# jhoobergs/Thesis-pbrt-v3

Measured on AMD Instinct MI355X. Metric: Mrays/s, higher is better.
Workload: dtype f32; 1 GPU; Sponza-class atrium STAND-IN (311,728 tris, matte+plastic, point light; the reference ships no Sponza geometry) 700x700, halton 1024 spp, path maxdepth 5, bvh; spp_total=1024, tiles=16x16 round-robin over 1 GPU(s), parallelism=tile-dp1, film_merge=none (single GPU)

## Files before the change

thesis-pbrt-v3_amd/csrc/capi_device.hip:

```cpp
#include <hip/hip_runtime.h>
#include <algorithm>
#include <chrono>
#include <cmath>
#include <cstring>
#include <functional>
#include <map>
#include <memory>
#include <string>
#include <vector>
#include "../../include/hprt.h"
#include "device/kernels.h"
#include "halton_tables.h"
#include "host_transform.h"
#include "hprt_internal.h"
#include "device_state.h"
#include "scene_layout.h"
#include "wide_bvh.h"

using namespace hprt;


namespace {

int CheckDevice(int device, int *chosen) {
// ... 179 lines not shown
        dv.voxFunc = sc->voxFunc.as<float>(); dv.voxCdf = sc->voxCdf.as<float>(); dv.voxFuncInt = sc->voxFuncInt.as<float>();
        sc->nVoxels = (uint32_t)nVox; sc->voxRows = (uint32_t)rows; sc->voxRowsUsed = 0;
        if (dense) LaunchVoxelDistributions(nullptr, dv, sc->voxRi.as<float>(), (uint32_t)nVox, sc->voxFunc.as<float>(), sc->voxCdf.as<float>(), sc->voxFuncInt.as<float>());
        else {
            HIP_TRY(sc->voxSlot.alloc(nVox * sizeof(int32_t)));
            HIP_TRY(hipMemset(sc->voxSlot.p, 0xff, nVox * sizeof(int32_t)));
            HIP_TRY(sc->voxRequest.alloc(nVox * sizeof(uint32_t)));
            HIP_TRY(sc->voxRequestCount.alloc(256));
            HIP_TRY(hipMemset(sc->voxRequestCount.p, 0, 256));
            dv.voxSlot = sc->voxSlot.as<int32_t>(); dv.voxRequest = sc->voxRequest.as<uint32_t>(); dv.voxRequestCount = sc->voxRequestCount.as<uint32_t>();
        }
        HIP_TRY(hipGetLastError());
        HIP_TRY(hipDeviceSynchronize());
    }
    HIP_TRY(hipHostMalloc((void **)&sc->hostCounts, (4096 + 256) * sizeof(uint32_t)));
    *out = sc.release();
    return HPRT_OK;
} catch (...) { return hprt::HandleException(); }

__attribute__((visibility("default"))) int hprt_debug_scene_walk(HprtScene *s) { return s && s->walk == HprtScene::Walk::Bvh && hprt::WideWalkInUse(s->dev) ? 1 : 0; }
__attribute__((visibility("default"))) int hprt_debug_shade_counts(HprtScene *s, int on, uint64_t *out2) {
    if (!s) return HPRT_E_INVALID;
    if (out2) { out2[0] = s->shadeDeferred; out2[1] = s->shadeRetried; }
    if (on && !s->shadeCountsOn) s->shadeDeferred = s->shadeRetried = 0;
    s->shadeCountsOn = on != 0;
    return HPRT_OK;
}
__attribute__((visibility("default"))) int hprt_debug_poison_workspace(HprtScene *s, int byte) { if (!s) return HPRT_E_INVALID; s->poisonByte = byte < 0 ? -1 : (byte & 255); return HPRT_OK; }
__attribute__((visibility("default"))) int hprt_debug_capture_rays(HprtScene *s, int bounce, int kind, float *d_out7, size_t cap) {
    if (!s || kind < 0 || kind > 2 || cap > 0x7fffffffull) return HPRT_E_INVALID;
    s->capture.bounce = bounce; s->capture.kind = kind; s->capture.out7 = d_out7; s->capture.cap = cap; s->capture.n = 0;
    return HPRT_OK;
}
static int ApiStreams(HprtScene *s, size_t n, RayStream *rays, HitStream *hits);
static bool CountsKdShare(const HprtScene *s) { return s->walk == HprtScene::Walk::RbspKd || s->walk == HprtScene::Walk::BspPaperKd; }
static void Trace(HprtScene *s, hipStream_t st, bool anyHit, bool count, const uint32_t *queue, const uint32_t *countPtr, uint32_t countImm,
                  uint32_t gridItems, const RayStream &rays, const HitStream &hits, uint8_t *occ, DevCounters *counters, uint32_t *workCounter,
                  uint4 *rayStats = nullptr) {
    switch (s->walk) {
    case HprtScene::Walk::Kd: LaunchKdTrace(st, s->dev, s->kd, anyHit, count, queue, countPtr, countImm, gridItems, rays, hits, occ, counters, workCounter, rayStats); break;
    case HprtScene::Walk::Rbsp: LaunchRbspTrace(st, s->dev, s->rbsp, anyHit, count, queue, countPtr, countImm, gridItems, rays, hits, occ, counters, workCounter, rayStats); break;
    case HprtScene::Walk::RbspKd:
        LaunchRbspKdTrace(st, s->dev, DevRbspKd{s->rbsp, s->kdShare.as<unsigned long long>()}, anyHit, count, queue, countPtr, countImm, gridItems, rays,
                          hits, occ, counters, workCounter, rayStats);
        break;
    case HprtScene::Walk::BspPaper:
        LaunchBspPaperTrace(st, s->dev, s->bsppaper, anyHit, count, queue, countPtr, countImm, gridItems, rays, hits, occ, counters, workCounter, rayStats);
        break;
    case HprtScene::Walk::BspPaperKd:
        LaunchBspPaperKdTrace(st, s->dev, DevBspPaperKd{s->bsppaper, s->kdShare.as<unsigned long long>()}, anyHit, count, queue, countPtr, countImm,
// ... 403 lines not shown
        HIP_TRY(outOcc.alloc(n));
        HitStream none; none.a = nullptr; none.b = nullptr;
        Trace(s, nullptr, true, count, nullptr, nullptr, (uint32_t)n, (uint32_t)n, rays, none, outOcc.as<uint8_t>(), s->counters.as<DevCounters>(), s->workCounter.as<uint32_t>());
        HIP_TRY(hipGetLastError()); HIP_TRY(hipDeviceSynchronize());
        if (occ_out) HIP_TRY(hipMemcpy(occ_out, outOcc.p, n, hipMemcpyDeviceToHost));
    }
    if (counters) ReadCounters(s, anyHit, counters);
    return HPRT_OK;
}
int hprt_intersect(HprtScene *s, size_t n, const float *o, const float *d, const float *tmax, float *t_out, int32_t *prim_out,
                   float *bary_out, uint64_t counters[4]) try {
    return TraceHost(s, false, n, o, d, tmax, t_out, prim_out, nullptr, bary_out, nullptr, counters);
} catch (...) { return hprt::HandleException(); }
int hprt_intersect_instanced(HprtScene *s, size_t n, const float *o, const float *d, const float *tmax, float *t_out, int32_t *prim_out,
                             int32_t *inst_out, float *bary_out, uint64_t counters[4]) try {
    return TraceHost(s, false, n, o, d, tmax, t_out, prim_out, inst_out, bary_out, nullptr, counters);
} catch (...) { return hprt::HandleException(); }
int hprt_occluded(HprtScene *s, size_t n, const float *o, const float *d, const float *tmax, uint8_t *occ, uint64_t counters[4]) try {
    return TraceHost(s, true, n, o, d, tmax, nullptr, nullptr, nullptr, nullptr, occ, counters);
} catch (...) { return hprt::HandleException(); }

namespace {

struct BatchTimers { double extendMs = 0, occludedMs = 0; uint64_t extendLaunches = 0, occludedLaunches = 0, extendRays = 0, occludedRays = 0; };

int RunBatch(HprtScene *s, hipStream_t st, const RenderParams &rp, const Workspace &w, const QueueSet &qa, const QueueSet &qb,
             const BinSet &bins, uint32_t s0, uint32_t nSlots, bool count, EventTimer &ev, BatchTimers *bt, HprtRenderStats *stats,
             uint32_t *pixelStats = nullptr, const IrregularSink *irregular = nullptr) {
    uint4 *rayStats = pixelStats ? s->rayStats.as<uint4>() : nullptr;
    uint32_t *pixelKd = pixelStats && CountsKdShare(s) ? s->pixelKdLocal.as<uint32_t>() : nullptr;
    uint32_t *wcPath = s->workCounter.as<uint32_t>();
    LaunchGenerate(st, s->dev, rp, w.path[0], s0, nSlots, irregular);
    const uint32_t *activeQ = nullptr; uint32_t active = nSlots;
    QueueSet q[2] = {qa, qb};
    DevCounters *ctr = s->counters.as<DevCounters>();
    std::vector<std::pair<hipEvent_t, hipEvent_t>> evExt, evOcc;
    auto tracePath = [&](int bounce) -> int {
        const PathStream &in = w.path[bounce & 1];
        hipEvent_t e0 = ev.get(), e1 = ev.get();
        HIP_TRY(hipEventRecord(e0, st));
        Trace(s, st, false, count, activeQ, nullptr, active, active, in.ray, w.hit, nullptr, ctr, wcPath, rayStats);
        if (pixelStats) LaunchPixelStats(st, rayStats, bounce == 0 ? nullptr : in.beta, activeQ, nullptr, active, active, rp.nPix, false, pixelStats);
        if (pixelKd) LaunchPixelKdStats(st, rayStats, bounce == 0 ? nullptr : in.beta, activeQ, nullptr, active, active, rp.nPix, false, pixelKd);
        HIP_TRY(hipEventRecord(e1, st));
        evExt.push_back({e0, e1}); bt->extendRays += active; ++bt->extendLaunches;
        stats->rays += active;
        return HPRT_OK;
    };
    if (active > 0) { int rc = tracePath(0); if (rc != HPRT_OK) return rc; }
    for (int bounce = 0; active > 0; ++bounce) {
        const QueueSet &cur = q[bounce & 1];
        const PathStream &in = w.path[bounce & 1], &out = w.path[(bounce + 1) & 1];
// ... 44 lines not shown
            hipEvent_t a = ev.get(), b = ev.get();
            HIP_TRY(hipEventRecord(a, st));
            HitStream none; none.a = nullptr; none.b = nullptr;
            Trace(s, st, true, count, cur.shadow, nullptr, nShadow, nShadow, w.vs.shadow, none, w.vs.occluded, ctr, wcPath, rayStats);
            if (pixelStats) LaunchPixelStats(st, rayStats, w.vs.pendBeta, cur.shadow, nullptr, nShadow, nShadow, rp.nPix, true, pixelStats);
            if (pixelKd) LaunchPixelKdStats(st, rayStats, w.vs.pendBeta, cur.shadow, nullptr, nShadow, nShadow, rp.nPix, true, pixelKd);
            HIP_TRY(hipEventRecord(b, st));
            evOcc.push_back({a, b}); bt->occludedRays += nShadow; ++bt->occludedLaunches;
            stats->shadow_rays += nShadow;
        }
        if (nMis) {
            hipEvent_t a = ev.get(), b = ev.get();
            HIP_TRY(hipEventRecord(a, st));
            Trace(s, st, false, count, cur.mis, nullptr, nMis, nMis, w.vs.mis, w.vs.misHit, nullptr, ctr, wcPath, rayStats);
            if (pixelStats) LaunchPixelStats(st, rayStats, w.vs.pendBeta, cur.mis, nullptr, nMis, nMis, rp.nPix, false, pixelStats);
            if (pixelKd) LaunchPixelKdStats(st, rayStats, w.vs.pendBeta, cur.mis, nullptr, nMis, nMis, rp.nPix, false, pixelKd);
            HIP_TRY(hipEventRecord(b, st));
            evExt.push_back({a, b}); bt->extendRays += nMis; ++bt->extendLaunches;
            stats->rays += nMis;
        }
        activeQ = cur.next; active = nNext;
        if (active > 0 && bounce > rp.maxDepth) return SetError(HPRT_E_DEVICE, "internal error: paths are still active beyond maxdepth");
        if (nResolve) LaunchResolve(st, s->dev, w.vs, out.L, w.Lfinal, cur.resolve, cur.resolveCount, nResolve);
        if (active > 0) { int rc = tracePath(bounce + 1); if (rc != HPRT_OK) return rc; }
    }
    HIP_TRY(hipGetLastError());
    HIP_TRY(hipStreamSynchronize(st));
    for (auto &p : evExt) { float ms = 0; if (hipEventElapsedTime(&ms, p.first, p.second) == hipSuccess) bt->extendMs += ms; }
    for (auto &p : evOcc) { float ms = 0; if (hipEventElapsedTime(&ms, p.first, p.second) == hipSuccess) bt->occludedMs += ms; }
    ev.reset();
    return HPRT_OK;
}

constexpr size_t kQueueWordsPerSlot = 8 + 1 + 2 * N_BINS;
int EnsureWorkspace(HprtScene *s, size_t nSlots, Workspace *ps, QueueSet *qa, QueueSet *qb, BinSet *bins) {
    HIP_TRY(s->planes.alloc(PlaneBytes(nSlots)));
    CarvePlanes(s->planes.as<char>(), nSlots, ps);
    HIP_TRY(s->queues.alloc(kQueueWordsPerSlot * nSlots * sizeof(uint32_t) + 4096));
    HIP_TRY(s->queueCounts.alloc(2048 * sizeof(uint32_t)));
    uint32_t *qbase = s->queues.as<uint32_t>(), *cbase = s->queueCounts.as<uint32_t>();
    QueueSet *qs[2] = {qa, qb};
    for (int k = 0; k < 2; ++k) {
        qs[k]->next = qbase + (4 * k + 0) * nSlots; qs[k]->shadow = qbase + (4 * k + 1) * nSlots;
        qs[k]->mis = qbase + (4 * k + 2) * nSlots; qs[k]->resolve = qbase + (4 * k + 3) * nSlots;
        qs[k]->nextCount = cbase + 256 * k; qs[k]->shadowCount = cbase + 256 * k + 64; qs[k]->misCount = cbase + 256 * k + 128; qs[k]->resolveCount = cbase + 256 * k + 192;
    }
    bins->aux = qbase + 8 * nSlots;
    for (int k = 0; k < (int)N_BINS; ++k) bins->q[k] = reinterpret_cast<uint2 *>(qbase + (9 + 2 * k) * nSlots + (nSlots & 1u));
    bins->count = cbase + 512;
    bins->retry[0] = bins->retry[1] = nullptr;
// ... 69 lines not shown
    HIP_TRY(hipMemsetAsync(film, 0, 16 * s->filmPixels, st));
    if (nPix == 0) { HIP_TRY(hipStreamSynchronize(st)); return HPRT_OK; }
    const size_t lallBytes = 3ull * spp * nPix * sizeof(float);
    if (lallBytes > (96ull << 30)) return SetError(HPRT_E_UNSUPPORTED, "per-sample radiance store would exceed 96 GiB; render in several tile ranges");
    uint32_t chunk = 0;
    if ((rc = ChooseBatch(s, desc->spp_chunk, nPix, spp, &chunk)) != HPRT_OK) return rc;
    const size_t maxSlots = (size_t)chunk * nPix;
    Workspace ps; QueueSet qa, qb; BinSet bins;
    rc = EnsureWorkspace(s, maxSlots, &ps, &qa, &qb, &bins);
    if (rc != HPRT_OK) return rc;
    HIP_TRY(s->Lall.alloc(lallBytes));
    if ((rc = PoisonWorkspace(s)) != HPRT_OK) return rc;
    float *LallR = s->Lall.as<float>(), *LallG = LallR + (size_t)spp * nPix, *LallB = LallG + (size_t)spp * nPix;
    HIP_TRY(upload(s->pixelXY, f.pixelXY)); HIP_TRY(upload(s->pixelOffset, f.pixelOffset));
    RenderParams rp;
    MakeCamera(o, &rp.cam);
    rp.hal.baseScale1 = f.hal.baseScales[1]; rp.hal.baseExp0 = f.hal.baseExponents[0]; rp.hal.sampleStride = f.hal.sampleStride;
    rp.hal.samplePixelCenter = o.sample_pixel_center;
    rp.pixelXY = s->pixelXY.as<uint32_t>(); rp.pixelOffset = s->pixelOffset.as<uint64_t>(); rp.nPix = nPix;
    rp.maxDepth = o.max_depth; rp.rrThreshold = o.rr_threshold;
    rp.invSqrtSpp = 1 / std::sqrt((float)spp);
    const bool wantPixelStats = (desc->flags & HPRT_RENDER_PIXEL_STATS) != 0;
    const bool count = (desc->flags & HPRT_RENDER_COUNT_WORK) != 0 || wantPixelStats;
    rp.cullMis = (!count || (desc->flags & HPRT_RENDER_COUNT_TRACED) != 0) && !(desc->flags & HPRT_RENDER_TRACE_ALL) ? 1 : 0;
    uint32_t *pixelStats = nullptr;
    if (wantPixelStats) {
        HIP_TRY(s->rayStats.alloc(sizeof(uint4) * maxSlots));
        HIP_TRY(s->pixelStatsLocal.alloc(6ull * nPix * sizeof(uint32_t)));
        HIP_TRY(hipMemsetAsync(s->pixelStatsLocal.p, 0, 6ull * nPix * sizeof(uint32_t), st));
        HIP_TRY(s->pixelStatsFilm.alloc(7ull * s->filmPixels * sizeof(uint64_t)));
        HIP_TRY(hipMemsetAsync(s->pixelStatsFilm.p, 0, 7ull * s->filmPixels * sizeof(uint64_t), st));
        pixelStats = s->pixelStatsLocal.as<uint32_t>();
        if (CountsKdShare(s)) {
            HIP_TRY(s->pixelKdLocal.alloc(2ull * nPix * sizeof(uint32_t)));
            HIP_TRY(hipMemsetAsync(s->pixelKdLocal.p, 0, 2ull * nPix * sizeof(uint32_t), st));
            HIP_TRY(s->pixelKdFilm.alloc(2ull * s->filmPixels * sizeof(uint64_t)));
            HIP_TRY(hipMemsetAsync(s->pixelKdFilm.p, 0, 2ull * s->filmPixels * sizeof(uint64_t), st));
        }
    }
    s->pixelStatsValid = false; s->pixelKdValid = false;
    HIP_TRY(hipMemsetAsync(s->counters.p, 0, sizeof(DevCounters), st));
    if (CountsKdShare(s)) HIP_TRY(hipMemsetAsync(s->kdShare.p, 0, 2 * sizeof(unsigned long long), st));

    auto wall0 = std::chrono::high_resolution_clock::now();
    static const uint32_t capHint = [] { const char *e = getenv("HPRT_IRREGULAR_CAP"); return e ? (uint32_t)std::max(1, atoi(e)) : (1u << 24); }();
    uint32_t irrCap = (uint32_t)std::min<uint64_t>((uint64_t)nPix * spp, capHint);
// ... 183 lines not shown
    SceneCall call(s, nullptr);
    FrameSetup f;
    int rc = SetupFrame(*opt, &f);
    if (rc != HPRT_OK) return rc;
    std::vector<uint32_t> xy(n); std::vector<uint64_t> off(n);
    for (size_t i = 0; i < n; ++i) {
        if (px[i] < f.fg.sx0 || px[i] >= f.fg.sx1 || py[i] < f.fg.sy0 || py[i] >= f.fg.sy1 || sample[i] < 0)
            return SetError(HPRT_E_INVALID, "hprt_sample_radiance: pixel outside the sample bounds");
        xy[i] = (uint32_t)px[i] | ((uint32_t)py[i] << 16);
        off[i] = (uint64_t)HaltonPixelOffset(f.hal, px[i], py[i]) + (uint64_t)sample[i] * (uint64_t)f.hal.sampleStride;
    }
    Workspace ps; QueueSet qa, qb; BinSet bins;
    rc = EnsureWorkspace(s, n, &ps, &qa, &qb, &bins);
    if (rc != HPRT_OK) return rc;
    HIP_TRY(upload(s->pixelXY, xy)); HIP_TRY(upload(s->pixelOffset, off));
    HIP_TRY(s->Lall.alloc(12 * n));
    if ((rc = PoisonWorkspace(s)) != HPRT_OK) return rc;
    RenderParams rp;
    MakeCamera(*opt, &rp.cam);
    rp.hal.baseScale1 = f.hal.baseScales[1]; rp.hal.baseExp0 = f.hal.baseExponents[0]; rp.hal.sampleStride = f.hal.sampleStride;
    rp.hal.samplePixelCenter = opt->sample_pixel_center;
    rp.pixelXY = s->pixelXY.as<uint32_t>(); rp.pixelOffset = s->pixelOffset.as<uint64_t>(); rp.nPix = (uint32_t)n;
    rp.maxDepth = opt->max_depth; rp.rrThreshold = opt->rr_threshold;
    rp.invSqrtSpp = 1 / std::sqrt((float)std::max(1, opt->spp)); rp.cullMis = 1;
    EventTimer ev; BatchTimers bt; HprtRenderStats stats; memset(&stats, 0, sizeof(stats));
    rc = RunBatch(s, nullptr, rp, ps, qa, qb, bins, 0, (uint32_t)n, false, ev, &bt, &stats);
    if (rc != HPRT_OK) return rc;
    float *LR = s->Lall.as<float>();
    LaunchStoreRadiance(nullptr, ps.Lfinal, LR, LR + n, LR + 2 * n, (uint32_t)n, 0, (uint32_t)n);
    HIP_TRY(hipGetLastError()); HIP_TRY(hipDeviceSynchronize());
    std::vector<float> planes(3 * n);
    HIP_TRY(hipMemcpy(planes.data(), LR, 12 * n, hipMemcpyDeviceToHost));
    for (size_t i = 0; i < n; ++i) { L_out[3 * i] = planes[i]; L_out[3 * i + 1] = planes[n + i]; L_out[3 * i + 2] = planes[2 * n + i]; }
    return HPRT_OK;
} catch (...) { return hprt::HandleException(); }

}
```

thesis-pbrt-v3_amd/csrc/device/kernels.h:

```cpp
#pragma once
#include <hip/hip_runtime.h>
#include <algorithm>
#include <type_traits>
#include "dev_shading.h"

namespace hprt {

struct RayStream { float4 *a, *b; };
struct HitStream { float4 *a; float2 *b; };
struct PathStream {
    RayStream ray;
    float4 *beta;
    float4 *L;
};
struct VertexStreams {
    RayStream shadow; uint8_t *occluded;
    RayStream mis; HitStream misHit;
    float4 *pendLight;
    float4 *pendMis;
    float4 *pendBeta;
};
struct QueueSet {
    uint32_t *next, *shadow, *mis, *resolve;
    uint32_t *nextCount, *shadowCount, *misCount, *resolveCount;
};
enum : uint32_t { BIN_STRIDE = 64u };
struct BinSet { uint2 *q[5]; uint32_t *aux; uint32_t *count; uint2 *retry[2]; };
struct RenderParams {
    DevCamera cam;
    DevHalton hal;
    const uint32_t *pixelXY;
    const uint64_t *pixelOffset;
    uint32_t nPix;
    int32_t maxDepth;
    float rrThreshold;
    float invSqrtSpp;
    int32_t cullMis;
};
struct FilmGeom {
    int32_t cx0, cy0, cx1, cy1;
    int32_t sx0, sy0, sx1, sy1;
    float rx, ry;
    float maxSampleLuminance;
};
struct IrregularSample { uint32_t pix, sample; int16_t x0, x1, y0, y1; };
struct IrregularSink { FilmGeom fg; uint32_t *count; uint32_t capacity; IrregularSample *out; };
struct FilmExtras {
    const uint32_t *ownBegin; const uint32_t *ownSrcPix; const uint32_t *ownSample; const uint8_t *ownIsPre;
    uint32_t nForeignDest;
    const uint32_t *foreignDestFilmIndex; const uint32_t *foreignDestBegin; const uint32_t *foreignGroupBegin;
    const uint32_t *foreignSrcPix; const uint32_t *foreignSample;
};

struct FilmRecord { uint32_t dest, srcTile; float xyz[3]; float w; };

bool WideWalkInUse(const DevScene &sc);
void LaunchTrace(hipStream_t st, const DevScene &sc, bool anyHit, bool count, const uint32_t *queue, const uint32_t *countPtr,
                 uint32_t countImm, uint32_t gridItems, const RayStream &rays, const HitStream &hits, uint8_t *occ,
                 DevCounters *counters, uint32_t *workCounter, uint4 *rayStats = nullptr);
template <uint32_t BLOCK, uint32_t WAVES, uint32_t QUAD_WAVES, typename Launch>
void LaunchTreeWalk(hipStream_t st, const DevScene &sc, bool anyHit, bool count, uint32_t gridItems, uint32_t *workCounter, Launch launch) {
    if (gridItems == 0) return;
    (void)hipMemsetAsync(workCounter, 0, sizeof(uint32_t), st);
    const bool quad = sc.nSpheres != 0u;
    const dim3 grid(std::min((uint32_t)(((size_t)gridItems + BLOCK - 1) / BLOCK), 256u * (quad ? QUAD_WAVES : WAVES))), block(BLOCK);
    auto pickQuad = [&](auto a, auto c) { if (quad) launch(grid, block, a, c, std::true_type{}); else launch(grid, block, a, c, std::false_type{}); };
    auto pickCount = [&](auto a) { if (count) pickQuad(a, std::true_type{}); else pickQuad(a, std::false_type{}); };
    if (anyHit) pickCount(std::true_type{}); else pickCount(std::false_type{});
}
void LaunchPixelStats(hipStream_t st, const uint4 *rayStats, const float4 *ids, const uint32_t *queue, const uint32_t *countPtr,
                      uint32_t countImm, uint32_t gridItems, uint32_t nPix, bool anyHit, uint32_t *pix);
void LaunchPixelStatsToFilm(hipStream_t st, const uint32_t *pix, const uint32_t *pixelXY, uint32_t nPix, uint32_t spp, int cx0, int cy0, int width,
                            unsigned long long *out7);
void LaunchGenerate(hipStream_t st, const DevScene &sc, const RenderParams &rp, const PathStream &out, uint32_t s0, uint32_t nSlots,
                    const IrregularSink *irr = nullptr);
void LaunchBin(hipStream_t st, const DevScene &sc, const PathStream &in, const HitStream &hit, const uint32_t *queue,
               const uint32_t *countPtr, uint32_t countImm, uint32_t gridItems, int32_t maxDepth, int32_t bounces, const BinSet &bins,
               float4 *Lfinal);
void LaunchShade(hipStream_t st, int mode, const DevScene &sc, const RenderParams &rp, const PathStream &in, const HitStream &hit,
                 uint32_t gridItems, uint32_t s0, const PathStream &out, const VertexStreams &vs, const QueueSet &q,
                 const BinSet &bins, float4 *Lfinal, bool firstBounce, bool retryPass = false);
void LaunchResolve(hipStream_t st, const DevScene &sc, const VertexStreams &vs, float4 *L, float4 *Lfinal, const uint32_t *queue,
                   const uint32_t *countPtr, uint32_t gridItems);
void LaunchStoreRadiance(hipStream_t st, const float4 *Lfinal, float *LallR, float *LallG, float *LallB, uint32_t nPix, uint32_t s0,
                         uint32_t nSlots);
void LaunchPackRays(hipStream_t st, const float *rays7, uint32_t n, const RayStream &out);
void LaunchUnpackHits(hipStream_t st, const HitStream &hits, uint32_t n, float *t, int32_t *prim, float *bary3);
void LaunchFindIrregular(hipStream_t st, const DevScene &sc, const RenderParams &rp, const FilmGeom &fg, uint32_t spp, uint32_t *count,
                         uint32_t capacity, IrregularSample *out);
void LaunchFilmOwn(hipStream_t st, const RenderParams &rp, const FilmGeom &fg, const float *LallR, const float *LallG, const float *LallB,
                   uint32_t spp, const FilmExtras &ex, float *film);
void LaunchFilmForeign(hipStream_t st, const RenderParams &rp, const FilmGeom &fg, const float *LallR, const float *LallG,
                       const float *LallB, const FilmExtras &ex, float *film);
void LaunchFilmForeignExport(hipStream_t st, const RenderParams &rp, const FilmGeom &fg, const float *LallR, const float *LallG,
                             const float *LallB, const FilmExtras &ex, uint32_t nGroups, const uint32_t *groupDest, const uint32_t *groupTile,
                             FilmRecord *out);
void LaunchVoxelDistributions(hipStream_t st, const DevScene &sc, const float *ri, uint32_t nVox, float *func, float *cdf, float *funcInt);
void LaunchVoxelFill(hipStream_t st, const DevScene &sc, const float *ri, uint32_t n, uint32_t rowBase, float *func, float *cdf, float *funcInt);
void LaunchStreamCopy(hipStream_t st, const float4 *src, float4 *dst, size_t n);
void LaunchGatherProbe(hipStream_t st, const uint4 *records, uint32_t log2Records, int itersPerLane, uint32_t blocks, uint32_t *sink);
void LaunchCaptureRays(hipStream_t st, const uint32_t *queue, uint32_t n, const RayStream &rays, float *out7, uint32_t cap);
void LaunchFilmApplyRecords(hipStream_t st, const FilmRecord *rec, const uint32_t *destBegin, uint32_t nDest, float *film);

}
```

thesis-pbrt-v3_amd/csrc/device/kernels.hip:

```cpp
#include <hip/hip_runtime.h>
#include <algorithm>
#include <cstdio>
#include <cstdlib>
#include <string>
#include "dev_shading.h"
#include "kernels.h"
#ifndef HPRT_QUAD_ANY_WAVES
#define HPRT_QUAD_ANY_WAVES 5
#endif
#define HPRT_QUAD_CLOSEST_WAVES 4
#ifndef HPRT_LDS_STACK_QUAD_ANY
#define HPRT_LDS_STACK_QUAD_ANY 12
#endif
#define HPRT_LDS_STACK_INST_ANY 7
#define HPRT_LDS_STACK_INST_CLOSEST 9
#ifndef HPRT_ANY_WAVES
#define HPRT_ANY_WAVES 7
#endif
#ifndef HPRT_CLOSEST_WAVES
#define HPRT_CLOSEST_WAVES 6
#endif
#ifndef HPRT_LDS_STACK_CLOSEST
#define HPRT_LDS_STACK_CLOSEST 12
#endif
// ... 930 lines not shown
#define HPRT_SHADE_WAVES_PLASTIC 4
#endif
#ifndef HPRT_SHADE_WAVES_GENERIC
#define HPRT_SHADE_WAVES_GENERIC 3
#endif
#ifndef HPRT_SHADE_WAVES_SUBSTRATE
#define HPRT_SHADE_WAVES_SUBSTRATE 4
#endif
template <int MODE, int BS, bool TEX = false, bool INSTS = false>
__global__ __launch_bounds__(BS, MODE == 0 ? HPRT_SHADE_WAVES_MATTE : MODE == 1 ? HPRT_SHADE_WAVES_PLASTIC : MODE == 3 ? HPRT_SHADE_WAVES_SUBSTRATE : HPRT_SHADE_WAVES_GENERIC) void k_shade(DevScene sc, RenderParams rp, PathStream in, HitStream hit, uint32_t s0,
                                               PathStream out, VertexStreams vs, QueueSet q, BinSet bins, float4 *Lfinal, uint32_t firstBounce, uint32_t retryPass) {
    __shared__ HaltonLds hl;
    __shared__ BlockAppendLds al;
    constexpr int BIN = MODE == 2 ? (TEX ? (int)BIN_TEXTURED : (int)BIN_GENERIC) : MODE == 3 ? (int)BIN_SUBSTRATE : MODE;
    constexpr int RETRY = BIN == (int)BIN_TEXTURED ? 1 : 0;
    const uint32_t n = retryPass ? bins.count[(6 + RETRY) * BIN_STRIDE] : bins.count[BIN * BIN_STRIDE];
    if (blockIdx.x * blockDim.x >= n) return;
    const uint32_t i = blockIdx.x * blockDim.x + threadIdx.x;
#ifdef HPRT_SHADE_PROF
    unsigned long long spT[8] = {0, 0, 0, 0, 0, 0, 0, 0}, spLast = clock64();
    bool spFull = false;
#endif
    bool wantNext = false, wantShadow = false, wantMis = false, wantResolve = false, defer = false, voxelMiss = false;
    uint32_t slot = 0;
    uint32_t j = 0;
    float4 rayA = make_float4(0.f, 0.f, 0.f, 0.f), rayB = rayA, hitA = rayA, beta4 = rayA, L4 = rayA, tv0 = rayA, tv1 = rayA, tv2 = rayA;
    float2 hitB = make_float2(0.f, __int_as_float(-1));
    int32_t word = -1;
    const bool oneLight = sc.nLights == 1u && !sc.spatial;
    DevLight light0 = {};
    if (oneLight) light0 = sc.lights[0];
    if (i < n) {
        const uint2 e = (retryPass ? bins.retry[RETRY] : bins.q[BIN])[i];
        slot = e.x;
        word = retryPass ? __float_as_int(hit.a[slot].y) : (int32_t)e.y;
        if (retryPass) j = e.y;
        else {
            j = (BIN == (int)BIN_MATTE ? 0u : BIN == (int)BIN_PLASTIC ? bins.count[0] : BIN == (int)BIN_SUBSTRATE ? bins.count[0] + bins.count[BIN_STRIDE]
                 : BIN == (int)BIN_GENERIC ? bins.count[0] + bins.count[BIN_STRIDE] + bins.count[4 * BIN_STRIDE]
                 : bins.count[0] + bins.count[BIN_STRIDE] + bins.count[4 * BIN_STRIDE] + bins.count[5 * BIN_STRIDE]) + i;
            if (BIN == (int)BIN_GENERIC && i >= bins.count[5 * BIN_STRIDE]) j = bins.aux[i];
        }
        const int32_t p = hit_prim(word);
        if (MODE != 2 || p >= 0) { tv0 = sc.tris[3 * p]; tv1 = sc.tris[3 * p + 1]; tv2 = sc.tris[3 * p + 2]; }
        hitA = hit.a[slot]; rayA = in.ray.a[slot]; rayB = in.ray.b[slot];
        if (hit.b) hitB = hit.b[slot];
        beta4 = firstBounce ? make_float4(1.f, 1.f, 1.f, __uint_as_float(slot)) : in.beta[slot];
        L4 = firstBounce ? make_float4(0.f, 0.f, 0.f, 1.f) : in.L[slot];
    }
    halton_lds_load(sc, &hl);
    if (i < n) {
        SP_MARK(6);
        const uint32_t st = __float_as_uint(rayB.w);
        int dim = (int)(st & 0xffffu);
        const int bounces = (int)((st >> 16) & 0x7fffu);
        const bool specularBounce = (st >> 31) != 0u;
        const uint32_t pathId = __float_as_uint(beta4.w);
        const uint32_t pix = pathId % rp.nPix, sIdx = pathId / rp.nPix;
        const uint64_t index = (uint64_t)rp.pixelOffset[pix] + (uint64_t)(s0 + sIdx) * (uint64_t)rp.hal.sampleStride;
        const int32_t prim = hit_prim(word);
        const vec3 rayO(rayA.x, rayA.y, rayA.z);
        const vec3 rayD(rayB.x, rayB.y, rayB.z);
        rgb beta(beta4.x, beta4.y, beta4.z);
        rgb L(L4.x, L4.y, L4.z);
        float etaScale = L4.w;
        const bool found = prim >= 0;
        DevSI si;
        DevTexGeom tg;
        constexpr bool texScene = MODE == 2 && TEX;
        if (found) {
            const float4 v0 = tv0;
            const int inst = (MODE == 2 || INSTS) ? __float_as_int(hitB.y) : -1;
            DRay r0; r0.o = rayO; r0.d = rayD; r0.tMax = rayA.w;
            if ((MODE == 2 || INSTS) && inst >= 0) {
                const DevInstance &in = sc.instances[inst];
                vec3 oErr;
                r0.o = xf_point_err(in.w2i, rayO, &oErr);
                r0.d = xf_vector(in.w2i, rayD);
                const float lengthSquared = r0.d.x * r0.d.x + r0.d.y * r0.d.y + r0.d.z * r0.d.z;
                if (lengthSquared > 0) {
                    const float dt = dot(vabs(r0.d), oErr) / lengthSquared;
                    r0.o = r0.o + r0.d * dt;
                    r0.tMax -= dt;
                }
            }
            if (MODE != 2 || (__float_as_uint(v0.w) & TAG_KIND_MASK) == 0u)
                fill_triangle(sc, (uint32_t)prim, tv0, tv1, tv2, hitA.z, hitA.w, hitB.x, r0.d, &si, texScene ? &tg : nullptr);
// ... 109 lines not shown
                        int sampledType = 0;
                        rgb f = bsdf_sample(bsdf, si.wo, &wi, us0, us1, &scatteringPdf, &sampledType);
                        f = f * absdot(wi, si.ns);
                        if (!is_black(f) && scatteringPdf > 0) {
                            const vec3 o = offset_ray_origin(si.p, si.pErr, si.n, wi);
                            DRay mr; mr.o = o; mr.d = wi; mr.tMax = HPRT_INF;
                            float tb0, tb1, tb2, tt;
                            if (!rp.cullMis || (MODE == 2 && light.type == 4) ||
                                (MODE == 2 && light.type == 3 ? triangle_may_hit(sc, light.prim, mr, &tb0, &tb1, &tb2, &tt)
                                                              : sphere_may_hit(sc.spheres[light.sphere], mr))) {
                                const float lp = light_pdf<MODE == 2>(sc, light, it, wi);
                                if (lp != 0) {
                                    const float w = power_heuristic(scatteringPdf, lp);
                                    vs.mis.a[j] = make_float4(o.x, o.y, o.z, HPRT_INF);
                                    vs.mis.b[j] = make_float4(wi.x, wi.y, wi.z, 0.f);
                                    rgb Lemit(light.I[0], light.I[1], light.I[2]);
                                    if (MODE == 2 && light.type == 4) Lemit = env_Le(sc, sc.envLights[light.shape], wi);
                                    pendMis = f * Lemit * rgb(1.f) * w / scatteringPdf;
                                    wantMis = true;
                                }
                            }
                        }
                    }
                    if (wantShadow || wantMis) {
                        vs.pendLight[j] = make_float4(pendLight.r, pendLight.g, pendLight.b,
                                                      __uint_as_float((uint32_t)lightNum | (wantShadow ? 0x40000000u : 0u) | (wantMis ? 0x80000000u : 0u)));
                        if (wantMis || sc.spatial) vs.pendMis[j] = make_float4(pendMis.r, pendMis.g, pendMis.b, pickPdf);
                        vs.pendBeta[j] = make_float4(beta.r, beta.g, beta.b, beta4.w);
                        wantResolve = true;
                    }
                    }
                }
            }
            if (!defer && !wantResolve && bsdf_num(bsdf) > 0) L = rgb(L.r + beta.r * 0.f, L.g + beta.g * 0.f, L.b + beta.b * 0.f);
            SP_MARK(4);
            if (!defer) {
            const float ub0 = halton_dim(sc, rp.hal, index, dim, &hl), ub1 = halton_dim(sc, rp.hal, index, dim + 1, &hl);
            dim += 2;
            vec3 wo = -rayD, wi;
            float pdf = 0; int flags = 0;
            rgb f = bsdf_sample(bsdf, wo, &wi, ub0, ub1, &pdf, &flags, true);
            if (!(is_black(f) || pdf == 0.f)) {
                beta = beta * (f * absdot(wi, si.ns) / pdf);
                vec3 o = offset_ray_origin(si.p, si.pErr, si.n, wi);
                bool alive = true;
                if (MODE == 2 && (flags & BX_SPECULAR) && (flags & BX_TRANSMISSION)) {
                    const float eta = bsdf.eta;
                    etaScale *= (dot(wo, si.n) > 0) ? (eta * eta) : 1 / (eta * eta);
                }
                rgb rrBeta = beta * etaScale;
                if (max_value(rrBeta) < rp.rrThreshold && bounces > 3) {
                    float qv = sel_max(.05f, 1 - max_value(rrBeta));
                    float u = halton_dim(sc, rp.hal, index, dim, &hl);
                    dim += 1;
                    if (u < qv) alive = false;
                    else beta = beta / (1 - qv);
                }
                if (rp.cullMis && bounces + 1 >= rp.maxDepth && !(flags & BX_SPECULAR)) alive = false;
                if (alive) {
                    out.ray.a[j] = make_float4(o.x, o.y, o.z, HPRT_INF);
                    out.ray.b[j] = make_float4(wi.x, wi.y, wi.z, __uint_as_float((uint32_t)dim | ((uint32_t)(bounces + 1) << 16) | ((flags & BX_SPECULAR) ? 0x80000000u : 0u)));
                    out.beta[j] = make_float4(beta.r, beta.g, beta.b, beta4.w);
                    wantNext = true;
                }
            }
            }
        }
        if (!defer) {
            if (wantNext || wantResolve) out.L[j] = make_float4(L.r, L.g, L.b, wantNext ? etaScale : 0.f);
            else Lfinal[pathId] = make_float4(L.r, L.g, L.b, 0.f);
        }
    }
    SP_MARK(5);
#ifdef HPRT_SHADE_PROF
    {
        const unsigned long long m = __ballot(spFull);
        if (m != 0ull && __lane_id() == (uint32_t)(__ffsll((long long)m) - 1)) {
            for (int k = 0; k < 7; ++k) atomicAdd(&g_shadeProf[MODE * 8 + k], spT[k]);
            atomicAdd(&g_shadeProf[MODE * 8 + 7], 1ull);
        }
    }
#endif
    if (MODE != 2) {
        const bool toGeneric = defer && !voxelMiss;
        const uint32_t p2 = wave_append(bins.count + 2 * BIN_STRIDE, toGeneric);
        if (toGeneric) { bins.q[2][p2] = make_uint2(slot, (uint32_t)word); bins.aux[p2] = j; }
    }
    if (sc.voxSlot) {
        const uint32_t pr = wave_append(bins.count + (6 + RETRY) * BIN_STRIDE, voxelMiss && !retryPass);
        if (voxelMiss && !retryPass) bins.retry[RETRY][pr] = make_uint2(slot, j);
    }
// ... 21 lines not shown
    const float pickPdf = sc.spatial ? pm.w : ((sc.lightFuncInt > 0) ? sc.lightFunc[lightNum] / (sc.lightFuncInt * (int)sc.nLights) : 0);
    rgb Ld(0.f);
    if ((info & 0x40000000u) && !vs.occluded[j]) Ld = Ld + rgb(pl.x, pl.y, pl.z);
    if (info & 0x80000000u) {
        const float4 mh = vs.misHit.a[j];
        const int32_t prim = hit_prim(__float_as_int(mh.y));
        if (prim < 0) {
            if (sc.lights[lightNum].type == 4) Ld = Ld + rgb(pm.x, pm.y, pm.z);
        } else if (prim_area_light(sc, prim) == lightNum) {
            const float4 ma = vs.mis.a[j], mb = vs.mis.b[j];
            DRay r; r.o = vec3(ma.x, ma.y, ma.z); r.d = vec3(mb.x, mb.y, mb.z); r.tMax = HPRT_INF;
            const DevLight light = sc.lights[lightNum];
            DevSI li;
            bool filled;
            if (light.type == 3) { fill_triangle(sc, (uint32_t)prim, mh.z, mh.w, vs.misHit.b[j].x, r.d, &li); filled = true; }
            else { float tt; filled = fill_sphere(sc, (int)__float_as_uint(sc.tris[3 * prim + 1].w), r, &li, &tt); }
            if (filled && (light.twoSided || dot(li.n, -r.d) > 0)) Ld = Ld + rgb(pm.x, pm.y, pm.z);
        }
    }
    rgb add = rgb(pb.x, pb.y, pb.z) * (Ld / pickPdf);
    const float4 Lnew = make_float4(L4.x + add.r, L4.y + add.g, L4.z + add.b, L4.w);
    if (L4.w != 0.f) Lio[j] = Lnew;
    else Lfinal[__float_as_uint(pb.w)] = Lnew;
}

__global__ __launch_bounds__(256) void k_store_radiance(const float4 *Lfinal, float *LallR, float *LallG, float *LallB, uint32_t nPix,
                                                         uint32_t s0, uint32_t nSlots) {
    const uint32_t slot = blockIdx.x * blockDim.x + threadIdx.x;
    if (slot >= nSlots) return;
    const float4 L4 = Lfinal[slot];
    rgb L(L4.x, L4.y, L4.z);
    const float y = luminance(L);
    if (is_nan(L.r) || is_nan(L.g) || is_nan(L.b)) L = rgb(0.f);
    else if ((double)y < -1e-5) L = rgb(0.f);
    else if (is_inf(y)) L = rgb(0.f);
    const size_t o = (size_t)s0 * nPix + slot;
    LallR[o] = L.r; LallG[o] = L.g; LallB[o] = L.b;
}

__global__ __launch_bounds__(256) void k_find_irregular(DevScene sc, RenderParams rp, FilmGeom fg, uint32_t spp, uint32_t *count,
                                                        uint32_t capacity, IrregularSample *out) {
    const size_t g = (size_t)blockIdx.x * blockDim.x + threadIdx.x;
    const size_t total = (size_t)rp.nPix * spp;
    bool irregular = false;
    IrregularSample rec;
    if (g < total) {
// ... 251 lines not shown
    static const int shadeCfg = [] {
        const char *e = getenv("HPRT_SHADE_BLOCK");
        const std::string v = e ? e : "512";
        return v == "1024" ? 0 : v == "256" ? 2 : 1;
    }();
    const bool specialised = mode == (int)BIN_MATTE || mode == (int)BIN_PLASTIC || mode == (int)BIN_SUBSTRATE;
    const uint32_t bs = !specialised ? 256u : (shadeCfg == 0 ? 1024u : shadeCfg == 1 ? 512u : 256u);
    dim3 grid(blocks_for(gridItems, bs)), block(bs);
#define HPRT_SHADE_LAUNCH_I(M, B, I) hipLaunchKernelGGL((k_shade<M, B, false, I>), grid, block, 0, st, sc, rp, in, hit, s0, out, vs, q, bins, Lfinal, firstBounce ? 1u : 0u, retryPass ? 1u : 0u)
#define HPRT_SHADE_LAUNCH(M, B) do { if (M != 2 && sc.nInstances != 0u) HPRT_SHADE_LAUNCH_I(M, B, (M != 2)); else HPRT_SHADE_LAUNCH_I(M, B, false); } while (0)
#define HPRT_SHADE_PICK(M) switch (shadeCfg) { case 0: HPRT_SHADE_LAUNCH(M, 1024); break; case 1: HPRT_SHADE_LAUNCH(M, 512); break; default: HPRT_SHADE_LAUNCH(M, 256); break; }
    if (mode == 3) hipLaunchKernelGGL((k_shade<2, 256, true>), grid, block, 0, st, sc, rp, in, hit, s0, out, vs, q, bins, Lfinal, firstBounce ? 1u : 0u, retryPass ? 1u : 0u);
    else if (mode == 2) { HPRT_SHADE_LAUNCH(2, 256); }
    else if (mode == 0) { HPRT_SHADE_PICK(0) }
    else if (mode == (int)BIN_SUBSTRATE) { HPRT_SHADE_PICK(3) }
    else { HPRT_SHADE_PICK(1) }
#undef HPRT_SHADE_PICK
#undef HPRT_SHADE_LAUNCH
}
void LaunchResolve(hipStream_t st, const DevScene &sc, const VertexStreams &vs, float4 *L, float4 *Lfinal, const uint32_t *queue,
                   const uint32_t *countPtr, uint32_t gridItems) {
    if (gridItems) hipLaunchKernelGGL(k_resolve, dim3(blocks_for(gridItems, 256)), dim3(256), 0, st, sc, vs, L, Lfinal, queue, countPtr);
}
void LaunchStoreRadiance(hipStream_t st, const float4 *Lfinal, float *LallR, float *LallG, float *LallB, uint32_t nPix, uint32_t s0,
                         uint32_t nSlots) {
    if (nSlots) hipLaunchKernelGGL(k_store_radiance, dim3(blocks_for(nSlots, 256)), dim3(256), 0, st, Lfinal, LallR, LallG, LallB, nPix, s0, nSlots);
}
__global__ __launch_bounds__(256) void k_pack_rays(const float *r7, uint32_t n, RayStream out) {
    const uint32_t i = blockIdx.x * blockDim.x + threadIdx.x;
    if (i >= n) return;
    const size_t N = n;
    out.a[i] = make_float4(r7[i], r7[N + i], r7[2 * N + i], r7[6 * N + i]);
    out.b[i] = make_float4(r7[3 * N + i], r7[4 * N + i], r7[5 * N + i], 0.f);
}
__global__ __launch_bounds__(256) void k_unpack_hits(HitStream h, uint32_t n, float *t, int32_t *prim, float *bary3) {
    const uint32_t i = blockIdx.x * blockDim.x + threadIdx.x;
    if (i >= n) return;
    const float4 a = h.a[i];
    t[i] = a.x; prim[i] = hit_prim(__float_as_int(a.y));
    if (bary3) { const size_t N = n; bary3[i] = a.z; bary3[N + i] = a.w; bary3[2 * N + i] = h.b[i].x; }
}
__global__ __launch_bounds__(256) void k_pixel_stats(const uint4 *rayStats, const float4 *ids, const uint32_t *queue, const uint32_t *countPtr,
                                                     uint32_t countImm, uint32_t nPix, int anyHit, uint32_t *pix) {
    const uint32_t n = countPtr ? *countPtr : countImm;
    const uint32_t i = blockIdx.x * blockDim.x + threadIdx.x;
    if (i >= n) return;
// ... 113 lines not shown
```

thesis-pbrt-v3_amd/csrc/device_state.h:

```cpp
#pragma once
#include <hip/hip_runtime.h>
#include <algorithm>
#include <mutex>
#include <string>
#include <vector>
#include "../../include/hprt.h"
#include "device/kernels.h"
#include "device/kd_walk.h"
#include "device/rbsp_walk.h"
#include "device/rbspkd_walk.h"
#include "device/bsppaper_walk.h"
#include "device/bsppaperkd_walk.h"
#include "device/kdinst_walk.h"
#include "hprt_internal.h"

#define HIP_TRY(expr)                                                                                   \
    do {                                                                                                \
        hipError_t e__ = (expr);                                                                        \
        if (e__ != hipSuccess)                                                                          \
            return hprt::SetError(HPRT_E_DEVICE, std::string(#expr) + ": " + hipGetErrorString(e__));   \
    } while (0)

namespace hprt {

// ... 19 lines not shown
}

struct HprtScene;
namespace hprt {
struct SceneCall {
    std::unique_lock<std::mutex> lk; HprtScene *s; hipStream_t st;
    SceneCall(HprtScene *scene, hipStream_t stream);
    void leave_async();
};
}

struct HprtScene {
    int device = 0;
    std::mutex mu;
    hipEvent_t lastUse = nullptr; bool lastUsePending = false;
    hprt::DevScene dev;
    hprt::DevBuf textures, mipLevels, texels, weightLut;
    hprt::DevBuf nodes, tris, primVtx, primN, vUV, vS, shapes, materials, lights, spheres, instances, topEntry, topEntryWide, lightFunc, lightCdf, perms, primes, primeSums, primeMagic;
    hprt::DevBuf envLights, envData;
    hprt::DevBuf wide, leafBox;
    hprt::DevBuf counters, workCounter, deepStack;
    struct Capture { int bounce = -1, kind = 0; float *out7 = nullptr; size_t cap = 0, n = 0; } capture;
    bool shadeCountsOn = false; uint64_t shadeDeferred = 0, shadeRetried = 0;
    int poisonByte = -1;
    hprt::DevBuf voxFunc, voxCdf, voxFuncInt, voxRi;
    hprt::DevBuf voxSlot, voxRequest, voxRequestCount, retryQueues;
    uint32_t voxRows = 0, voxRowsUsed = 0, nVoxels = 0;
    hprt::DevBuf rayStats, pixelStatsLocal, pixelStatsFilm; bool pixelStatsValid = false;
    hprt::DevBuf planes;
    hprt::DevBuf apiRays, apiHits;
    hprt::DevBuf queues, queueCounts;
    hprt::DevBuf pixelXY, pixelOffset, Lall, film, irregular, irregularCount;
    hprt::DevBuf exOwnBegin, exOwnSrc, exOwnSample, exOwnPre, exFDest, exFDestBegin, exFGroupBegin, exFSrc, exFSample;
    hprt::DevBuf foreignRecords, exGroupDest, exGroupTile; uint32_t nForeignRecords = 0; bool foreignExported = false;
    int filmW = 0, filmH = 0;
    float *lastFilm = nullptr;
    uint32_t *hostCounts = nullptr;
    size_t filmPixels = 0;
    uint32_t nPrims = 0;
    enum class Walk { Bvh, Kd, Rbsp, RbspKd, BspPaper, BspPaperKd, KdInst } walk = Walk::Bvh;
    hprt::DevBuf treeNodes, treePrims, treeAxes; hprt::DevKd kd{}; hprt::DevRbsp rbsp{}; hprt::DevBspPaper bsppaper{};
    hprt::DevBuf kdShare, pixelKdLocal, pixelKdFilm; bool pixelKdValid = false;
    std::vector<uint32_t> topOrder; bool instanced = false;
    bool hasSubstrateBin = false;
    hprt::DevBuf kdInstEntries; hprt::DevKdInst kdinst{};
    std::vector<std::vector<uint32_t>> objectOrder; std::vector<uint32_t> objectPrimBase; std::vector<int32_t> instanceObject;
// ... 12 lines not shown
```

Before: 6024 Mrays/s.

## Speculatively add direct light in shade and repair occluded paths afterward

For shadow-only light samples (no MIS), the shade kernel now adds the direct-light contribution to the path radiance up front. It also stores the unlit radiance in pendBeta as a repair record. After the occlusion trace, a small repair kernel restores the unlit value only for occluded rays. This removes the separate resolve pass and its pending-light and MIS writes for unoccluded rays, at the cost of an extra kernel launch, one extra record write per shadow ray, and reuse of the pendBeta buffer.

```diff
diff --git a/thesis-pbrt-v3_amd/csrc/capi_device.hip b/thesis-pbrt-v3_amd/csrc/capi_device.hip
--- a/thesis-pbrt-v3_amd/csrc/capi_device.hip
+++ b/thesis-pbrt-v3_amd/csrc/capi_device.hip
@@ -1,5 +1,6 @@
 #include <hip/hip_runtime.h>
 #include <algorithm>
+#include <cassert>
 #include <chrono>
 #include <cmath>
 #include <cstring>
@@ -225,10 +226,21 @@
 __attribute__((visibility("default"))) int hprt_debug_shade_counts(HprtScene *s, int on, uint64_t *out2) {
     if (!s) return HPRT_E_INVALID;
     if (out2) { out2[0] = s->shadeDeferred; out2[1] = s->shadeRetried; }
-    if (on && !s->shadeCountsOn) s->shadeDeferred = s->shadeRetried = 0;
+    if (on && !s->shadeCountsOn) s->shadeDeferred = s->shadeRetried = s->shadeSpeculated = s->shadeRepaired = s->shadeFull = 0;
     s->shadeCountsOn = on != 0;
     return HPRT_OK;
 }
+__attribute__((visibility("default"))) int hprt_debug_speculated_counts(HprtScene *s, uint64_t *out3) {
+    if (!s || !out3) return HPRT_E_INVALID;
+    out3[0] = s->shadeSpeculated; out3[1] = s->shadeRepaired; out3[2] = s->shadeFull;
+    return HPRT_OK;
+}
+static int g_speculateLight = -1;
+static bool SpeculateLightEnabled() {
+    static const bool fromEnv = [] { const char *e = getenv("HPRT_SPECULATE_LIGHT"); return !(e && atoi(e) == 0); }();
+    return g_speculateLight < 0 ? fromEnv : g_speculateLight != 0;
+}
+__attribute__((visibility("default"))) int hprt_debug_speculate_light(int on) { const int was = SpeculateLightEnabled() ? 1 : 0; g_speculateLight = on; return was; }
 __attribute__((visibility("default"))) int hprt_debug_poison_workspace(HprtScene *s, int byte) { if (!s) return HPRT_E_INVALID; s->poisonByte = byte < 0 ? -1 : (byte & 255); return HPRT_OK; }
 __attribute__((visibility("default"))) int hprt_debug_capture_rays(HprtScene *s, int bounce, int kind, float *d_out7, size_t cap) {
     if (!s || kind < 0 || kind > 2 || cap > 0x7fffffffull) return HPRT_E_INVALID;
@@ -678,12 +690,18 @@
 
 namespace {
 
+constexpr size_t kSpecCountsAt = 1024;
 struct BatchTimers { double extendMs = 0, occludedMs = 0; uint64_t extendLaunches = 0, occludedLaunches = 0, extendRays = 0, occludedRays = 0; };
 
-int RunBatch(HprtScene *s, hipStream_t st, const RenderParams &rp, const Workspace &w, const QueueSet &qa, const QueueSet &qb,
+int RunBatch(HprtScene *s, hipStream_t st, const RenderParams &rpIn, const Workspace &w, const QueueSet &qa, const QueueSet &qb,
              const BinSet &bins, uint32_t s0, uint32_t nSlots, bool count, EventTimer &ev, BatchTimers *bt, HprtRenderStats *stats,
              uint32_t *pixelStats = nullptr, const IrregularSink *irregular = nullptr) {
     uint4 *rayStats = pixelStats ? s->rayStats.as<uint4>() : nullptr;
+    RenderParams rp = rpIn;
+    rp.speculate = SpeculateLightEnabled() && !pixelStats && !rayStats && nSlots <= SPEC_MAX_PATHS ? 1 : 0;
+    assert(!rp.speculate || nSlots <= SPEC_MAX_PATHS);
+    uint32_t *specCounts = rp.speculate && s->shadeCountsOn ? s->queueCounts.as<uint32_t>() + kSpecCountsAt : nullptr;
+    if (specCounts) HIP_TRY(hipMemsetAsync(specCounts, 0, 2 * sizeof(uint32_t), st));
     uint32_t *pixelKd = pixelStats && CountsKdShare(s) ? s->pixelKdLocal.as<uint32_t>() : nullptr;
     uint32_t *wcPath = s->workCounter.as<uint32_t>();
     LaunchGenerate(st, s->dev, rp, w.path[0], s0, nSlots, irregular);
@@ -774,10 +792,14 @@
         activeQ = cur.next; active = nNext;
         if (active > 0 && bounce > rp.maxDepth) return SetError(HPRT_E_DEVICE, "internal error: paths are still active beyond maxdepth");
         if (nResolve) LaunchResolve(st, s->dev, w.vs, out.L, w.Lfinal, cur.resolve, cur.resolveCount, nResolve);
+        if (rp.speculate && nShadow) LaunchRepair(st, w.vs, out.L, w.Lfinal, cur.shadow, nShadow, specCounts);
+        if (s->shadeCountsOn) s->shadeFull += nResolve;
         if (active > 0) { int rc = tracePath(bounce + 1); if (rc != HPRT_OK) return rc; }
     }
     HIP_TRY(hipGetLastError());
+    if (specCounts) HIP_TRY(hipMemcpyAsync(s->hostCounts + 256, specCounts, 2 * sizeof(uint32_t), hipMemcpyDeviceToHost, st));
     HIP_TRY(hipStreamSynchronize(st));
+    if (specCounts) { s->shadeSpeculated += s->hostCounts[256]; s->shadeRepaired += s->hostCounts[257]; }
     for (auto &p : evExt) { float ms = 0; if (hipEventElapsedTime(&ms, p.first, p.second) == hipSuccess) bt->extendMs += ms; }
     for (auto &p : evOcc) { float ms = 0; if (hipEventElapsedTime(&ms, p.first, p.second) == hipSuccess) bt->occludedMs += ms; }
     ev.reset();
@@ -893,6 +915,7 @@
     rp.invSqrtSpp = 1 / std::sqrt((float)spp);
     const bool wantPixelStats = (desc->flags & HPRT_RENDER_PIXEL_STATS) != 0;
     const bool count = (desc->flags & HPRT_RENDER_COUNT_WORK) != 0 || wantPixelStats;
+    rp.speculate = 0;
     rp.cullMis = (!count || (desc->flags & HPRT_RENDER_COUNT_TRACED) != 0) && !(desc->flags & HPRT_RENDER_TRACE_ALL) ? 1 : 0;
     uint32_t *pixelStats = nullptr;
     if (wantPixelStats) {
@@ -1122,7 +1145,7 @@
     rp.hal.samplePixelCenter = opt->sample_pixel_center;
     rp.pixelXY = s->pixelXY.as<uint32_t>(); rp.pixelOffset = s->pixelOffset.as<uint64_t>(); rp.nPix = (uint32_t)n;
     rp.maxDepth = opt->max_depth; rp.rrThreshold = opt->rr_threshold;
-    rp.invSqrtSpp = 1 / std::sqrt((float)std::max(1, opt->spp)); rp.cullMis = 1;
+    rp.invSqrtSpp = 1 / std::sqrt((float)std::max(1, opt->spp)); rp.cullMis = 1; rp.speculate = 0;
     EventTimer ev; BatchTimers bt; HprtRenderStats stats; memset(&stats, 0, sizeof(stats));
     rc = RunBatch(s, nullptr, rp, ps, qa, qb, bins, 0, (uint32_t)n, false, ev, &bt, &stats);
     if (rc != HPRT_OK) return rc;
diff --git a/thesis-pbrt-v3_amd/csrc/device/kernels.h b/thesis-pbrt-v3_amd/csrc/device/kernels.h
--- a/thesis-pbrt-v3_amd/csrc/device/kernels.h
+++ b/thesis-pbrt-v3_amd/csrc/device/kernels.h
@@ -20,6 +20,7 @@
     float4 *pendMis;
     float4 *pendBeta;
 };
+enum : uint32_t { SPEC_RECORD = 0x80000000u, SPEC_END = 0x40000000u, SPEC_ID_MASK = 0x0fffffffu, SPEC_MAX_PATHS = 1u << 28 };
 struct QueueSet {
     uint32_t *next, *shadow, *mis, *resolve;
     uint32_t *nextCount, *shadowCount, *misCount, *resolveCount;
@@ -36,6 +37,7 @@
     float rrThreshold;
     float invSqrtSpp;
     int32_t cullMis;
+    int32_t speculate;
 };
 struct FilmGeom {
     int32_t cx0, cy0, cx1, cy1;
@@ -82,6 +84,7 @@
                  const BinSet &bins, float4 *Lfinal, bool firstBounce, bool retryPass = false);
 void LaunchResolve(hipStream_t st, const DevScene &sc, const VertexStreams &vs, float4 *L, float4 *Lfinal, const uint32_t *queue,
                    const uint32_t *countPtr, uint32_t gridItems);
+void LaunchRepair(hipStream_t st, const VertexStreams &vs, float4 *L, float4 *Lfinal, const uint32_t *queue, uint32_t n, uint32_t *counts);
 void LaunchStoreRadiance(hipStream_t st, const float4 *Lfinal, float *LallR, float *LallG, float *LallB, uint32_t nPix, uint32_t s0,
                          uint32_t nSlots);
 void LaunchPackRays(hipStream_t st, const float *rays7, uint32_t n, const RayStream &out);
diff --git a/thesis-pbrt-v3_amd/csrc/device/kernels.hip b/thesis-pbrt-v3_amd/csrc/device/kernels.hip
--- a/thesis-pbrt-v3_amd/csrc/device/kernels.hip
+++ b/thesis-pbrt-v3_amd/csrc/device/kernels.hip
@@ -976,6 +976,7 @@
     bool spFull = false;
 #endif
     bool wantNext = false, wantShadow = false, wantMis = false, wantResolve = false, defer = false, voxelMiss = false;
+    bool speculated = false;
     uint32_t slot = 0;
     uint32_t j = 0;
     float4 rayA = make_float4(0.f, 0.f, 0.f, 0.f), rayB = rayA, hitA = rayA, beta4 = rayA, L4 = rayA, tv0 = rayA, tv1 = rayA, tv2 = rayA;
@@ -1016,7 +1017,7 @@
         const vec3 rayO(rayA.x, rayA.y, rayA.z);
         const vec3 rayD(rayB.x, rayB.y, rayB.z);
         rgb beta(beta4.x, beta4.y, beta4.z);
-        rgb L(L4.x, L4.y, L4.z);
+        rgb L(L4.x, L4.y, L4.z), Ldark(0.f);
         float etaScale = L4.w;
         const bool found = prim >= 0;
         DevSI si;
@@ -1172,7 +1173,14 @@
                             }
                         }
                     }
-                    if (wantShadow || wantMis) {
+                    if (rp.speculate && wantShadow && !wantMis) {
+                        rgb LdLit(0.f);
+                        LdLit = LdLit + pendLight;
+                        const rgb addLit = beta * (LdLit / pickPdf), addDark = beta * (rgb(0.f) / pickPdf);
+                        Ldark = rgb(L.r + addDark.r, L.g + addDark.g, L.b + addDark.b);
+                        L = rgb(L.r + addLit.r, L.g + addLit.g, L.b + addLit.b);
+                        speculated = true;
+                    } else if (wantShadow || wantMis) {
                         vs.pendLight[j] = make_float4(pendLight.r, pendLight.g, pendLight.b,
                                                       __uint_as_float((uint32_t)lightNum | (wantShadow ? 0x40000000u : 0u) | (wantMis ? 0x80000000u : 0u)));
                         if (wantMis || sc.spatial) vs.pendMis[j] = make_float4(pendMis.r, pendMis.g, pendMis.b, pickPdf);
@@ -1182,7 +1190,7 @@
                     }
                 }
             }
-            if (!defer && !wantResolve && bsdf_num(bsdf) > 0) L = rgb(L.r + beta.r * 0.f, L.g + beta.g * 0.f, L.b + beta.b * 0.f);
+            if (!defer && !wantResolve && !speculated && bsdf_num(bsdf) > 0) L = rgb(L.r + beta.r * 0.f, L.g + beta.g * 0.f, L.b + beta.b * 0.f);
             SP_MARK(4);
             if (!defer) {
             const float ub0 = halton_dim(sc, rp.hal, index, dim, &hl), ub1 = halton_dim(sc, rp.hal, index, dim + 1, &hl);
@@ -1217,6 +1225,7 @@
             }
         }
         if (!defer) {
+            if (speculated) vs.pendBeta[j] = make_float4(Ldark.r, Ldark.g, Ldark.b, __uint_as_float(pathId | SPEC_RECORD | (wantNext ? 0u : SPEC_END)));
             if (wantNext || wantResolve) out.L[j] = make_float4(L.r, L.g, L.b, wantNext ? etaScale : 0.f);
             else Lfinal[pathId] = make_float4(L.r, L.g, L.b, 0.f);
         }
@@ -1284,6 +1293,26 @@
     const float4 Lnew = make_float4(L4.x + add.r, L4.y + add.g, L4.z + add.b, L4.w);
     if (L4.w != 0.f) Lio[j] = Lnew;
     else Lfinal[__float_as_uint(pb.w)] = Lnew;
+}
+
+template <bool COUNT>
+__global__ __launch_bounds__(256) void k_repair(VertexStreams vs, float4 *Lio, float4 *Lfinal, const uint32_t *queue, uint32_t n, uint32_t *counts) {
+    const uint32_t i = blockIdx.x * blockDim.x + threadIdx.x;
+    if (i >= n) return;
+    const uint32_t j = queue[i];
+    const bool occluded = vs.occluded[j] != 0;
+    if (!COUNT && !occluded) return;
+    const float4 rec = vs.pendBeta[j];
+    const uint32_t w = __float_as_uint(rec.w);
+    if (!(w & SPEC_RECORD)) return;
+    if (COUNT) atomicAdd(counts, 1u);
+    if (!occluded) return;
+    if (COUNT) atomicAdd(counts + 1, 1u);
+    if (w & SPEC_END) Lfinal[w & SPEC_ID_MASK] = make_float4(rec.x, rec.y, rec.z, 0.f);
+    else {
+        float *const Lj = reinterpret_cast<float *>(Lio + j);
+        Lj[0] = rec.x; Lj[1] = rec.y; Lj[2] = rec.z;
+    }
 }
 
 __global__ __launch_bounds__(256) void k_store_radiance(const float4 *Lfinal, float *LallR, float *LallG, float *LallB, uint32_t nPix,
@@ -1581,6 +1610,11 @@
                    const uint32_t *countPtr, uint32_t gridItems) {
     if (gridItems) hipLaunchKernelGGL(k_resolve, dim3(blocks_for(gridItems, 256)), dim3(256), 0, st, sc, vs, L, Lfinal, queue, countPtr);
 }
+void LaunchRepair(hipStream_t st, const VertexStreams &vs, float4 *L, float4 *Lfinal, const uint32_t *queue, uint32_t n, uint32_t *counts) {
+    if (n == 0) return;
+    if (counts) hipLaunchKernelGGL(k_repair<true>, dim3(blocks_for(n, 256)), dim3(256), 0, st, vs, L, Lfinal, queue, n, counts);
+    else hipLaunchKernelGGL(k_repair<false>, dim3(blocks_for(n, 256)), dim3(256), 0, st, vs, L, Lfinal, queue, n, counts);
+}
 void LaunchStoreRadiance(hipStream_t st, const float4 *Lfinal, float *LallR, float *LallG, float *LallB, uint32_t nPix, uint32_t s0,
                          uint32_t nSlots) {
     if (nSlots) hipLaunchKernelGGL(k_store_radiance, dim3(blocks_for(nSlots, 256)), dim3(256), 0, st, Lfinal, LallR, LallG, LallB, nPix, s0, nSlots);
diff --git a/thesis-pbrt-v3_amd/csrc/device_state.h b/thesis-pbrt-v3_amd/csrc/device_state.h
--- a/thesis-pbrt-v3_amd/csrc/device_state.h
+++ b/thesis-pbrt-v3_amd/csrc/device_state.h
@@ -65,6 +65,7 @@
     hprt::DevBuf counters, workCounter, deepStack;
     struct Capture { int bounce = -1, kind = 0; float *out7 = nullptr; size_t cap = 0, n = 0; } capture;
     bool shadeCountsOn = false; uint64_t shadeDeferred = 0, shadeRetried = 0;
+    uint64_t shadeSpeculated = 0, shadeRepaired = 0, shadeFull = 0;
     int poisonByte = -1;
     hprt::DevBuf voxFunc, voxCdf, voxFuncInt, voxRi;
     hprt::DevBuf voxSlot, voxRequest, voxRequestCount, retryQueues;
```

Measured after the change: 6203 Mrays/s (median of 6 runs). 3.0% higher.
